# olegroshka/vae-channel-dynamics

Hardware: AMD Instinct MI355X
Metric: images/sec SDXL-VAE train step @256x256 (tracking on) (higher is better)
Workload: dtype f32

## Files before the change

### vae-channel-dynamics_amd/csrc/conv3_upwino.hip

```cpp
#include "wino_common.h"
#include <type_traits>
#include <algorithm>

#ifndef VAE_UPW_PRIO
#define VAE_UPW_PRIO 1
#endif
#ifndef VAE_UPW_XCD_LIMIT
#define VAE_UPW_XCD_LIMIT (4 << 20)
#endif
#ifndef VAE_UPW_X3
#define VAE_UPW_X3 1
#endif
#if VAE_UPW_X3
#include "bf16_frag.h"
#endif

namespace {

constexpr int UTH = 4, UTW = 8;
constexpr int UTL = UTH * UTW;
static_assert(UTL == wino::TILES, "spill_acc");
constexpr int NPOS = 9;
constexpr int UNT = 512;
constexpr int UNB = 2;
constexpr int UHF = (UTH + 2) * (UTW + 2);
constexpr int UHD = (2 * UTH + 2) * (2 * UTW + 2);
constexpr int UMLD = 33;
constexpr int USM = NPOS * UTL * UMLD;

#if !VAE_UPW_X3
constexpr int UBK = 8;
constexpr int USV = NPOS * UTL * UBK;
constexpr int USH = UHD * UBK;
constexpr int UP_LDS = (USM > 2 * USV + 2 * USH ? USM : 2 * USV + 2 * USH) * 4;

__global__ __launch_bounds__(256) void upwino_weights_kernel(const float* __restrict__ W, int N, int K, int dgrad, int64_t sn, int64_t sk, int64_t st,
                                                             float* __restrict__ U) {
  const int64_t i = (int64_t)blockIdx.x * 256 + threadIdx.x;
  if (i >= (int64_t)N * K) return;
  const int k = (int)(i % K), n = (int)(i / K);
  float g[3][3];
  wino::u_gather(W, n, k, dgrad, sn, sk, st, g);
  float t[3][3];
#pragma unroll
  for (int b = 0; b < 3; ++b) {
    t[0][b] = g[0][b];
    t[1][b] = (g[0][b] + g[2][b]) + g[1][b];
    t[2][b] = g[2][b];
  }
  float* o = wino::u_out<NPOS>(U, N, n, k);
#pragma unroll
  for (int a = 0; a < 3; ++a) {
    wino::u_at(o, N, a * 3 + 0) = t[a][0];
    wino::u_at(o, N, a * 3 + 1) = (t[a][0] + t[a][2]) + t[a][1];
    wino::u_at(o, N, a * 3 + 2) = t[a][2];
  }
}

template <bool DG>
__global__ __launch_bounds__(UNT, 4) void conv3_upwino_kernel(vae_igemm_args p, const float* __restrict__ U, int tiles_x, int tiles_y, int xcd_sp) {
  constexpr int WBN = 32 * UNB;
  constexpr int HW_ = DG ? 2 * UTW + 2 : UTW + 2;
  constexpr int HP = DG ? UHD : UHF;
  __shared__ __attribute__((aligned(16))) float wsm[UP_LDS / 4];
  float* const sV = wsm;
  float* const sH = wsm + 2 * USV;

  const int tid = threadIdx.x, lane = tid & 63, wave = tid >> 6;
  const int xw0 = (blockIdx.x & 1) * 2;
  const bool extra = wave == xw0 || wave == xw0 + 1;
  const int xnb = wave - xw0;
  const int lr = lane & 31, lh = lane >> 5;
  const vae_conv_geom g = p.g;
  const int tilesN = (p.N + WBN - 1) / WBN;
  const wino::TileId wg = wino::tile_of_workgroup(blockIdx.x, tilesN, tiles_x, tiles_y, xcd_sp);
  const int b = wg.b;
  const int y0 = wg.ty * UTH, x0 = wg.tx * UTW, n0 = wg.tn * WBN;
  const int nsteps = p.K / UBK;

  const bool hrole = tid < 2 * HP;
  const int hp = tid >> 1, hq = tid & 1;
  const int hy = (DG ? 2 * y0 : y0) - 1 + hp / HW_, hx = (DG ? 2 * x0 : x0) - 1 + hp % HW_;
  const bool hin = hrole && ((unsigned)hy < (unsigned)g.Hs) && ((unsigned)hx < (unsigned)g.Ws);
  const auto rsA = VAE_BUF_RSRC(p.A + (int64_t)b * g.Hs * g.Ws * g.Cs, (size_t)g.Hs * g.Ws * g.Cs * 4u);
  const unsigned hbase = hin ? (unsigned)(((hy * g.Ws + hx) * g.Cs + hq * 4) * 4) : BUF_OOB;
  f32x4 rh = {0.f, 0.f, 0.f, 0.f};
  auto load_halo_into = [&](int step, f32x4& h) {
    const bool ok = hin && step < nsteps;
    h = VAE_BUF_LOAD4(rsA, ok ? hbase + (unsigned)(step * UBK * 4) : BUF_OOB);
  };
  auto store_halo_from = [&](float* dst, const f32x4& h) {
    if (hrole) *reinterpret_cast<f32x4*>(&dst[hp * UBK + hq * 4]) = h;
  };

  const bool vrole = tid < 256;
  const int vt = (tid >> 3) & 31, vc = tid & 7;
  const int vorg = DG ? ((2 * (vt >> 3)) * HW_ + 2 * (vt & 7)) * UBK + vc : ((vt >> 3) * HW_ + (vt & 7)) * UBK + vc;
  auto write_v = [&](const float* sHc, float* dst) {
    if (!vrole) return;
    float r[3][DG ? 4 : 3];
    if (!DG) {
      float d[3][3];
#pragma unroll
      for (int i = 0; i < 3; ++i)
#pragma unroll
        for (int j = 0; j < 3; ++j) d[i][j] = sHc[vorg + (i * HW_ + j) * UBK];
#pragma unroll
      for (int j = 0; j < 3; ++j) {
        r[0][j] = d[0][j] - d[1][j];
        r[1][j] = d[1][j];
        r[2][j] = d[1][j] - d[2][j];
      }
#pragma unroll
      for (int a = 0; a < 3; ++a) {
        dst[((a * 3 + 0) * UTL + vt) * UBK + vc] = r[a][0] - r[a][1];
        dst[((a * 3 + 1) * UTL + vt) * UBK + vc] = r[a][1];
        dst[((a * 3 + 2) * UTL + vt) * UBK + vc] = r[a][1] - r[a][2];
      }
    } else {
      float d[4][4];
#pragma unroll
      for (int i = 0; i < 4; ++i)
#pragma unroll
        for (int j = 0; j < 4; ++j) d[i][j] = sHc[vorg + (i * HW_ + j) * UBK];
#pragma unroll
      for (int j = 0; j < 4; ++j) {
        r[0][j] = d[0][j] - d[2][j];
        r[1][j] = d[1][j] + d[2][j];
        r[2][j] = d[1][j] - d[3][j];
      }
#pragma unroll
      for (int a = 0; a < 3; ++a) {
        dst[((a * 3 + 0) * UTL + vt) * UBK + vc] = r[a][0] - r[a][2];
        dst[((a * 3 + 1) * UTL + vt) * UBK + vc] = r[a][1] + r[a][2];
        dst[((a * 3 + 2) * UTL + vt) * UBK + vc] = r[a][1] - r[a][3];
      }
    }
  };

  const auto rsU = VAE_BUF_RSRC(U, wino::u_bytes(nsteps, NPOS, p.N));
  unsigned bvo[UNB];
#pragma unroll
  for (int q = 0; q < UNB; ++q) bvo[q] = (n0 + q * 32 + lr < p.N) ? wino::u_frag(n0 + q * 32 + lr, lh) : BUF_OOB;
  const unsigned bpos = wino::u_pos_bytes(p.N);
  const unsigned bvx = extra ? bvo[xnb & 1] : BUF_OOB;
  f32x4 bq[UNB + 1];
  auto load_b1 = [&](int step, int i) {
    const int st = min(step, nsteps - 1);
    const unsigned so = __builtin_amdgcn_readfirstlane((unsigned)(st * NPOS + (i < UNB ? wave : 8)) * bpos);
    bq[i] = __builtin_bit_cast(f32x4, __builtin_amdgcn_raw_buffer_load_b128(rsU, i < UNB ? bvo[i < UNB ? i : 0] : bvx, so, 0));
  };

  f32x16 acc[UNB], accx;
#pragma unroll
  for (int nb = 0; nb < UNB; ++nb)
#pragma unroll
    for (int e = 0; e < 16; ++e) acc[nb][e] = 0.f;
#pragma unroll
  for (int e = 0; e < 16; ++e) accx[e] = 0.f;

#pragma unroll
  for (int i = 0; i <= UNB; ++i) load_b1(0, i);
  {
    f32x4 h0, h1;
    load_halo_into(0, h0);
    load_halo_into(1, h1);
    load_halo_into(2, rh);
    store_halo_from(sH, h0);
    store_halo_from(sH + USH, h1);
  }
  __syncthreads();
  write_v(sH, sV);
  __syncthreads();
  auto multiply = [&](const float* cV, int s) {
    const f32x4 a4 = *reinterpret_cast<const f32x4*>(&cV[(wave * UTL + lr) * UBK + 4 * lh]);
    f32x4 ax = a4;
    if (extra) ax = *reinterpret_cast<const f32x4*>(&cV[(8 * UTL + lr) * UBK + 4 * lh]);
#pragma unroll
    for (int nb = 0; nb < UNB; ++nb) {
#pragma unroll
      for (int e = 0; e < 4; ++e) acc[nb] = __builtin_amdgcn_mfma_f32_32x32x2f32(a4[e], bq[nb][e], acc[nb], 0, 0, 0);
      __builtin_amdgcn_sched_barrier(0);
      load_b1(s + 1, nb);
      __builtin_amdgcn_sched_barrier(0);
    }
    if (extra) {
#pragma unroll
      for (int e = 0; e < 4; ++e) accx = __builtin_amdgcn_mfma_f32_32x32x2f32(ax[e], bq[UNB][e], accx, 0, 0, 0);
    }
    __builtin_amdgcn_sched_barrier(0);
    load_b1(s + 1, UNB);
    __builtin_amdgcn_sched_barrier(0);
  };
  auto stage_next = [&](int s, int par) {
    if (s + 1 < nsteps) write_v(sH + (par ^ 1) * USH, sV + (par ^ 1) * USV);
    store_halo_from(sH + par * USH, rh);
    load_halo_into(s + 3, rh);
  };
  auto step = [&](int s, int par, auto first_c) {
    const float* cV = sV + par * USV;
    if (decltype(first_c)::value) {
      stage_next(s, par);
      __builtin_amdgcn_sched_barrier(0);
      multiply(cV, s);
    } else {
      multiply(cV, s);
      __builtin_amdgcn_sched_barrier(0);
      stage_next(s, par);
    }
    __syncthreads();
  };
  auto run = [&](auto first_c) {
    int s = 0;
    for (; s + 1 < nsteps; s += 2) {
      step(s, 0, first_c);
      step(s + 1, 1, first_c);
    }
    if (s < nsteps) step(s, 0, first_c);
  };
#if VAE_UPW_PRIO
  if (DG && __builtin_amdgcn_readfirstlane(tid) >= 256) __builtin_amdgcn_s_setprio(1);
#endif
  if (wave < 4) run(std::true_type{});
  else run(std::false_type{});
#if VAE_UPW_PRIO
  if (DG) __builtin_amdgcn_s_setprio(0);
#endif

  float* const sM = wsm;
  const size_t obytes = (size_t)g.Ho * g.Wo * p.ldc * 4u;
  const auto rsC = VAE_BUF_RSRC(p.C + (int64_t)b * g.Ho * g.Wo * p.ldc, obytes);
#pragma unroll
  for (int nb = 0; nb < UNB; ++nb) {
    if (nb > 0) __syncthreads();
    wino::spill_acc(sM, wave, UMLD, acc[nb], lr, lh);
    if (wave == xw0 + nb) wino::spill_acc(sM, 8, UMLD, accx, lr, lh);
    __syncthreads();
    {
#pragma unroll
      for (int rnd = 0; rnd < 2; ++rnd) {
        const int co = tid & 31, tile = (tid >> 5) + 16 * rnd;
        const int col = n0 + nb * 32 + co;
        float m[9];
#pragma unroll
        for (int pos = 0; pos < 9; ++pos) m[pos] = sM[(pos * UTL + tile) * UMLD + co];
        const int oy = y0 + (tile >> 3), ox = x0 + (tile & 7);
        if (!DG) {
          const float bv = (p.bias && col < p.N) ? p.bias[col] : 0.f;
          float h[2][3];
#pragma unroll
          for (int j = 0; j < 3; ++j) {
            h[0][j] = m[0 * 3 + j] + m[1 * 3 + j];
            h[1][j] = m[1 * 3 + j] - m[2 * 3 + j];
          }
#pragma unroll
          for (int a = 0; a < 2; ++a) {
            const float yv[2] = {h[a][0] + h[a][1], h[a][1] - h[a][2]};
#pragma unroll
            for (int bb = 0; bb < 2; ++bb) {
              const int py = 2 * oy + a, px = 2 * ox + bb;
              const unsigned off = (col < p.N && py < g.Ho && px < g.Wo) ? (unsigned)(((py * g.Wo + px) * p.ldc + col) * 4) : BUF_OOB;
              __builtin_amdgcn_raw_buffer_store_b32(__builtin_bit_cast(unsigned, yv[bb] + bv), rsC, off, 0, 0);
            }
          }
        } else {
          const float h0 = (m[0] + m[3]) - m[6], h1 = (m[1] + m[4]) - m[7], h2 = (m[2] + m[5]) - m[8];
          const float v = (h0 + h1) - h2;
          const unsigned off = (col < p.N && oy < g.Ho && ox < g.Wo) ? (unsigned)(((oy * g.Wo + ox) * p.ldc + col) * 4) : BUF_OOB;
          __builtin_amdgcn_raw_buffer_store_b32(__builtin_bit_cast(unsigned, v), rsC, off, 0, 0);
        }
      }
    }
  }
}

#else
constexpr int XBK = 16;
constexpr int XPL = NPOS * UTL * XBK;
constexpr int XSV = 3 * XPL;
template <bool DG>
constexpr int upw_lds_bytes() {
  constexpr int used = 2 * XSV * 2 + 2 * (DG ? UHD : UHF) * XBK * 4;
  return used > USM * 4 ? used : USM * 4;
}
extern __shared__ __attribute__((aligned(16))) float upw_lds[];

__host__ __device__ __forceinline__ int upw_chunks(int K) { return (K + XBK - 1) / XBK; }
__host__ __device__ __forceinline__ unsigned upw_plane_bytes(int N) { return (unsigned)N * (XBK * 2u); }
__host__ __device__ __forceinline__ size_t upw_u_bytes(int K, int N) { return (size_t)upw_chunks(K) * NPOS * 3 * upw_plane_bytes(N); }

__device__ __forceinline__ void upw_u_transform(const float (&g)[3][3], float (&o)[9]) {
  float t[3][3];
#pragma unroll
  for (int b = 0; b < 3; ++b) {
    t[0][b] = g[0][b];
    t[1][b] = (g[0][b] + g[2][b]) + g[1][b];
    t[2][b] = g[2][b];
  }
#pragma unroll
  for (int a = 0; a < 3; ++a) {
    o[a * 3 + 0] = t[a][0];
    o[a * 3 + 1] = (t[a][0] + t[a][2]) + t[a][1];
    o[a * 3 + 2] = t[a][2];
  }
}

__global__ __launch_bounds__(256) void upwino_weights_kernel(const float* __restrict__ W, int N, int K, int dgrad, int64_t sn, int64_t sk, int64_t st,
                                                             u16* __restrict__ U) {
  const int K16 = upw_chunks(K) * XBK;
  const int64_t i = (int64_t)blockIdx.x * 256 + threadIdx.x;
  if (i >= (int64_t)N * K16) return;
  const int k = (int)(i % K16), n = (int)(i / K16);
  float u[9];
  if (k < K) {
    float g[3][3];
    wino::u_gather(W, n, k, dgrad, sn, sk, st, g);
    upw_u_transform(g, u);
  } else {
#pragma unroll
    for (int pos = 0; pos < 9; ++pos) u[pos] = 0.f;
  }
  u16* o = U + ((int64_t)(k >> 4) * NPOS * 3 * N + n) * XBK + (k & 15);
#pragma unroll
  for (int pos = 0; pos < 9; ++pos) {
    unsigned hi, mid, lo;
    split3_pair(u[pos], 0.f, hi, mid, lo);
    o[(int64_t)(pos * 3 + 0) * N * XBK] = (u16)hi;
    o[(int64_t)(pos * 3 + 1) * N * XBK] = (u16)mid;
    o[(int64_t)(pos * 3 + 2) * N * XBK] = (u16)lo;
  }
}

template <bool DG>
__global__ __launch_bounds__(UNT, 4) void conv3_upwino_kernel(vae_igemm_args p, const u16* __restrict__ U, int tiles_x, int tiles_y, int xcd_sp) {
  constexpr int WBN = 32 * UNB;
  constexpr int HW_ = DG ? 2 * UTW + 2 : UTW + 2;
  constexpr int HP = DG ? UHD : UHF;
  constexpr int XSH = HP * XBK;
  u16* const sV = reinterpret_cast<u16*>(upw_lds);
  float* const sH = upw_lds + XSV;

  const int tid = threadIdx.x, lane = tid & 63, wave = tid >> 6;
  const int xw0 = (blockIdx.x & 1) * 2;
  const bool extra = wave == xw0 || wave == xw0 + 1;
  const int xnb = wave - xw0;
  const int lr = lane & 31, lh = lane >> 5;
  const vae_conv_geom g = p.g;
  const int tilesN = (p.N + WBN - 1) / WBN;
  const wino::TileId wg = wino::tile_of_workgroup(blockIdx.x, tilesN, tiles_x, tiles_y, xcd_sp);
  const int b = wg.b;
  const int y0 = wg.ty * UTH, x0 = wg.tx * UTW, n0 = wg.tn * WBN;
  const int nsteps = upw_chunks(p.K);

  const bool hrole = tid < 2 * HP;
  const int hp = tid >> 1, hq = tid & 1;
  const int hy = (DG ? 2 * y0 : y0) - 1 + hp / HW_, hx = (DG ? 2 * x0 : x0) - 1 + hp % HW_;
  const bool hin = hrole && ((unsigned)hy < (unsigned)g.Hs) && ((unsigned)hx < (unsigned)g.Ws);
  const auto rsA = VAE_BUF_RSRC(p.A + (int64_t)b * g.Hs * g.Ws * g.Cs, (size_t)g.Hs * g.Ws * g.Cs * 4u);
  const unsigned hbase = hin ? (unsigned)(((hy * g.Ws + hx) * g.Cs + hq * 8) * 4) : BUF_OOB;
  f32x4 rh[2] = {{0.f, 0.f, 0.f, 0.f}, {0.f, 0.f, 0.f, 0.f}};
  auto load_halo_into = [&](int step, f32x4 (&h)[2]) {
    const bool ok = hin && step * XBK + hq * 8 < p.K;
    h[0] = VAE_BUF_LOAD4(rsA, ok ? hbase + (unsigned)(step * XBK * 4) : BUF_OOB);
    h[1] = VAE_BUF_LOAD4(rsA, ok ? hbase + (unsigned)(step * XBK * 4 + 16) : BUF_OOB);
  };
  auto store_halo_from = [&](float* dst, const f32x4 (&h)[2]) {
    if (hrole) {
      *reinterpret_cast<f32x4*>(&dst[hp * XBK + hq * 8]) = h[0];
      *reinterpret_cast<f32x4*>(&dst[hp * XBK + hq * 8 + 4]) = h[1];
    }
  };

  const bool vrole = tid < 256;
  const int vt = (tid >> 3) & 31, vc = tid & 7;
  const int vorg = DG ? ((2 * (vt >> 3)) * HW_ + 2 * (vt & 7)) * XBK + 2 * vc : ((vt >> 3) * HW_ + (vt & 7)) * XBK + 2 * vc;
  const int vdst = vt * XBK + (((vc >> 2) ^ ((vt >> 3) & 1)) * 8) + (vc & 3) * 2;
  auto write_v = [&](const float* sHc, u16* dst) __attribute__((always_inline)) {
    if (!vrole) return;
    typedef float f32x2 __attribute__((ext_vector_type(2)));
    constexpr int NJ = DG ? 4 : 3;
#pragma unroll
    for (int a = 0; a < 3; ++a) {
      const int ia = DG ? (a == 0 ? 0 : 1) : (a == 0 ? 0 : 1), ib = DG ? (a == 2 ? 3 : 2) : (a == 0 ? 1 : 2);
      float r[NJ][2];
#pragma unroll
      for (int j = 0; j < NJ; ++j) {
        const f32x2 x = *reinterpret_cast<const f32x2*>(&sHc[vorg + (ia * HW_ + j) * XBK]);
        if (!DG && a == 1) {
          r[j][0] = x[0];
          r[j][1] = x[1];
        } else {
          const f32x2 y = *reinterpret_cast<const f32x2*>(&sHc[vorg + (ib * HW_ + j) * XBK]);
          const bool add = DG && a == 1;
          r[j][0] = add ? x[0] + y[0] : x[0] - y[0];
          r[j][1] = add ? x[1] + y[1] : x[1] - y[1];
        }
      }
      float o[3][2];
#pragma unroll
      for (int c = 0; c < 2; ++c) {
        if (!DG) {
          o[0][c] = r[0][c] - r[1][c];
          o[1][c] = r[1][c];
          o[2][c] = r[1][c] - r[2][c];
        } else {
          o[0][c] = r[0][c] - r[2][c];
          o[1][c] = r[1][c] + r[2][c];
          o[2][c] = r[1][c] - r[NJ - 1][c];
        }
      }
#pragma unroll
      for (int bb = 0; bb < 3; ++bb) {
        const int pos = a * 3 + bb;
        unsigned hi, mid, lo;
        split3_pair(o[bb][0], o[bb][1], hi, mid, lo);
        *reinterpret_cast<unsigned*>(&dst[0 * XPL + pos * UTL * XBK + vdst]) = hi;
        *reinterpret_cast<unsigned*>(&dst[1 * XPL + pos * UTL * XBK + vdst]) = mid;
        *reinterpret_cast<unsigned*>(&dst[2 * XPL + pos * UTL * XBK + vdst]) = lo;
      }
    }
  };

  const auto rsU = VAE_BUF_RSRC(U, upw_u_bytes(p.K, p.N));
  unsigned bvo[UNB];
#pragma unroll
  for (int q = 0; q < UNB; ++q) bvo[q] = (n0 + q * 32 + lr < p.N) ? (unsigned)(((n0 + q * 32 + lr) * XBK + lh * 8) * 2) : BUF_OOB;
  const unsigned bpl = upw_plane_bytes(p.N);
  const unsigned bvx = extra ? bvo[xnb & 1] : BUF_OOB;
  bf16x8 bq[UNB + 1][3];
  auto load_b3 = [&](int step, int i) __attribute__((always_inline)) {
    const int st = min(step, nsteps - 1);
    const unsigned so = __builtin_amdgcn_readfirstlane((unsigned)((st * NPOS + (i < UNB ? wave : 8)) * 3) * bpl);
#pragma unroll
    for (int pl = 0; pl < 3; ++pl)
      bq[i][pl] = __builtin_bit_cast(bf16x8, __builtin_amdgcn_raw_buffer_load_b128(rsU, i < UNB ? bvo[i < UNB ? i : 0] : bvx, so + (unsigned)pl * bpl, 0));
  };

  f32x16 acc[UNB], accx;
#pragma unroll
  for (int nb = 0; nb < UNB; ++nb)
#pragma unroll
    for (int e = 0; e < 16; ++e) acc[nb][e] = 0.f;
#pragma unroll
  for (int e = 0; e < 16; ++e) accx[e] = 0.f;

#pragma unroll
  for (int i = 0; i <= UNB; ++i) load_b3(0, i);
  {
    f32x4 h0[2], h1[2];
    load_halo_into(0, h0);
    load_halo_into(1, h1);
    load_halo_into(2, rh);
    store_halo_from(sH, h0);
    store_halo_from(sH + XSH, h1);
  }
  __syncthreads();
  write_v(sH, sV);
  __syncthreads();
  const int afrag = lr * XBK + ((lh ^ ((lr >> 3) & 1)) * 8);
  auto multiply = [&](const u16* cV, int s) __attribute__((always_inline)) {
    bf16x8 a[3];
#pragma unroll
    for (int pl = 0; pl < 3; ++pl) a[pl] = frag_direct(&cV[pl * XPL + wave * UTL * XBK + afrag]);
#pragma unroll
    for (int nb = 0; nb < UNB; ++nb) {
#pragma unroll
      for (int t = 0; t < 6; ++t) acc[nb] = mma_x3_term(t, a, bq[nb], acc[nb]);
      __builtin_amdgcn_sched_barrier(0);
      load_b3(s + 1, nb);
      __builtin_amdgcn_sched_barrier(0);
    }
    if (extra) {
#pragma unroll
      for (int pl = 0; pl < 3; ++pl) a[pl] = frag_direct(&cV[pl * XPL + 8 * UTL * XBK + afrag]);
#pragma unroll
      for (int t = 0; t < 6; ++t) accx = mma_x3_term(t, a, bq[UNB], accx);
    }
    __builtin_amdgcn_sched_barrier(0);
    load_b3(s + 1, UNB);
    __builtin_amdgcn_sched_barrier(0);
  };
  auto stage_next = [&](int s, int par) __attribute__((always_inline)) {
    store_halo_from(sH + par * XSH, rh);
    if (s + 1 < nsteps) write_v(sH + (par ^ 1) * XSH, sV + (par ^ 1) * XSV);
    load_halo_into(s + 3, rh);
  };
  auto step = [&](int s, int par, auto first_c) __attribute__((always_inline)) {
    const u16* cV = sV + par * XSV;
    if (decltype(first_c)::value) {
      stage_next(s, par);
      __builtin_amdgcn_sched_barrier(0);
      multiply(cV, s);
    } else {
      multiply(cV, s);
      __builtin_amdgcn_sched_barrier(0);
      stage_next(s, par);
    }
    __syncthreads();
  };
  auto run = [&](auto first_c) __attribute__((always_inline)) {
    int s = 0;
    for (; s + 1 < nsteps; s += 2) {
      step(s, 0, first_c);
      step(s + 1, 1, first_c);
    }
    if (s < nsteps) step(s, 0, first_c);
  };
#if VAE_UPW_PRIO
  if (DG && __builtin_amdgcn_readfirstlane(tid) >= 256) __builtin_amdgcn_s_setprio(1);
#endif
  if (wave < 4) run(std::true_type{});
  else run(std::false_type{});
#if VAE_UPW_PRIO
  if (DG) __builtin_amdgcn_s_setprio(0);
#endif

  float* const sM = upw_lds;
  const size_t obytes = (size_t)g.Ho * g.Wo * p.ldc * 4u;
  const auto rsC = VAE_BUF_RSRC(p.C + (int64_t)b * g.Ho * g.Wo * p.ldc, obytes);
#pragma unroll
  for (int nb = 0; nb < UNB; ++nb) {
    if (nb > 0) __syncthreads();
    wino::spill_acc(sM, wave, UMLD, acc[nb], lr, lh);
    if (wave == xw0 + nb) wino::spill_acc(sM, 8, UMLD, accx, lr, lh);
    __syncthreads();
    {
#pragma unroll
      for (int rnd = 0; rnd < 2; ++rnd) {
        const int co = tid & 31, tile = (tid >> 5) + 16 * rnd;
        const int col = n0 + nb * 32 + co;
        float m[9];
#pragma unroll
        for (int pos = 0; pos < 9; ++pos) m[pos] = sM[(pos * UTL + tile) * UMLD + co];
        const int oy = y0 + (tile >> 3), ox = x0 + (tile & 7);
        if (!DG) {
          const float bv = (p.bias && col < p.N) ? p.bias[col] : 0.f;
          float h[2][3];
#pragma unroll
          for (int j = 0; j < 3; ++j) {
            h[0][j] = m[0 * 3 + j] + m[1 * 3 + j];
            h[1][j] = m[1 * 3 + j] - m[2 * 3 + j];
          }
#pragma unroll
          for (int a = 0; a < 2; ++a) {
            const float yv[2] = {h[a][0] + h[a][1], h[a][1] - h[a][2]};
#pragma unroll
            for (int bb = 0; bb < 2; ++bb) {
              const int py = 2 * oy + a, px = 2 * ox + bb;
              const unsigned off = (col < p.N && py < g.Ho && px < g.Wo) ? (unsigned)(((py * g.Wo + px) * p.ldc + col) * 4) : BUF_OOB;
              __builtin_amdgcn_raw_buffer_store_b32(__builtin_bit_cast(unsigned, yv[bb] + bv), rsC, off, 0, 0);
            }
          }
        } else {
          const float h0 = (m[0] + m[3]) - m[6], h1 = (m[1] + m[4]) - m[7], h2 = (m[2] + m[5]) - m[8];
          const float v = (h0 + h1) - h2;
          const unsigned off = (col < p.N && oy < g.Ho && ox < g.Wo) ? (unsigned)(((oy * g.Wo + ox) * p.ldc + col) * 4) : BUF_OOB;
          __builtin_amdgcn_raw_buffer_store_b32(__builtin_bit_cast(unsigned, v), rsC, off, 0, 0);
        }
      }
    }
  }
}
#endif

}

bool conv3_upwino_eligible(const vae_igemm_args& a) {
  const vae_conv_geom& g = a.g;
  if (!wino::conv_eligible_common(a, NPOS) || a.xf != VAE_XF_NONE) return false;
  if (a.track != nullptr || a.res != nullptr || a.gstat != nullptr || a.a_bf16 || a.res_bf16) return false;
  int Hl, Wl;
  if (g.mode == VAE_MODE_UP2X) {
    if (g.Ho != 2 * g.Hs || g.Wo != 2 * g.Ws || a.sk != 1) return false;
    Hl = g.Hs; Wl = g.Ws;
  } else if (g.mode == VAE_MODE_UP2X_DGRAD) {
    if (g.Hs != 2 * g.Ho || g.Ws != 2 * g.Wo || a.sn != 1 || a.bias != nullptr) return false;
    Hl = g.Ho; Wl = g.Wo;
  } else {
    return false;
  }
  if (Hl % UTH != 0 || Wl % UTW != 0 || a.K % 8 != 0 || a.K < 64 || a.K > 1024 || a.N < 32 || a.N % 4 != 0 || g.Cs < a.K) return false;
#if VAE_UPW_X3
  if (upw_u_bytes(a.K, a.N) >= BUF_MAX) return false;
#endif
  return true;
}

int64_t conv3_upwino_weight_bytes(const vae_igemm_args& a) {
#if VAE_UPW_X3
  return (int64_t)upw_u_bytes(a.K, a.N);
#else
  return (int64_t)wino::u_bytes(a.K / UBK, NPOS, a.N);
#endif
}

int launch_upwino_weights(const vae_igemm_args& a, float* U, hipStream_t st) {
#if VAE_UPW_X3
  const int64_t n = (int64_t)a.N * upw_chunks(a.K) * XBK;
  hipLaunchKernelGGL(upwino_weights_kernel, dim3((unsigned)((n + 255) / 256)), dim3(256), 0, st, a.W, a.N, a.K, a.g.mode == VAE_MODE_UP2X_DGRAD ? 1 : 0,
                     a.sn, a.sk, a.st, reinterpret_cast<u16*>(U));
  return 0;
#else
  return wino::launch_weights(upwino_weights_kernel, a, a.g.mode == VAE_MODE_UP2X_DGRAD, U, st);
#endif
}

int launch_conv3_upwino(const vae_igemm_args& a, const float* U, hipStream_t st) {
  const vae_conv_geom& g = a.g;
  const bool dg = g.mode == VAE_MODE_UP2X_DGRAD;
  const int Hl = dg ? g.Ho : g.Hs, Wl = dg ? g.Wo : g.Ws;
  const int tx = Wl / UTW, ty = Hl / UTH;
  const int tilesN = (a.N + 32 * UNB - 1) / (32 * UNB);
  const int64_t nt = (int64_t)tilesN * tx * ty * g.B;
  if (nt > 0x7fffffffLL) return VAE_EINVAL;
  constexpr size_t xcd_u = (size_t)VAE_UPW_XCD_LIMIT;
  const int xcd_sp = wino::xcd_spatial(tilesN, (size_t)conv3_upwino_weight_bytes(a), xcd_u, (int64_t)tx * ty * g.B);
#if VAE_UPW_X3
  const u16* Up = reinterpret_cast<const u16*>(U);
  if (dg) {
    VAE_RESERVE_LDS(conv3_upwino_kernel<true>, upw_lds_bytes<true>(), "conv3_upwino");
    hipLaunchKernelGGL((conv3_upwino_kernel<true>), dim3((unsigned)nt), dim3(UNT), upw_lds_bytes<true>(), st, a, Up, tx, ty, xcd_sp);
  } else {
    VAE_RESERVE_LDS(conv3_upwino_kernel<false>, upw_lds_bytes<false>(), "conv3_upwino");
    hipLaunchKernelGGL((conv3_upwino_kernel<false>), dim3((unsigned)nt), dim3(UNT), upw_lds_bytes<false>(), st, a, Up, tx, ty, xcd_sp);
  }
#else
  if (dg) hipLaunchKernelGGL((conv3_upwino_kernel<true>), dim3((unsigned)nt), dim3(UNT), 0, st, a, U, tx, ty, xcd_sp);
  else hipLaunchKernelGGL((conv3_upwino_kernel<false>), dim3((unsigned)nt), dim3(UNT), 0, st, a, U, tx, ty, xcd_sp);
#endif
  return 0;
}
```

Measured before the change: 118.8.

## Widen upsample Winograd conv N-tile to four 32-column blocks per workgroup

Makes the number of 32-wide output-channel blocks per workgroup configurable and defaults both forward and dgrad to 4 instead of 2. Each workgroup now reuses its transformed input tile across twice as many output channels, which halves the number of workgroups along N and cuts redundant input halo loads and V transforms. Waves 4-7 take the ninth Winograd position for the extra blocks, and partially live N tiles are masked. In exchange, accumulator register pressure doubles, so launch bounds drop to 2 blocks per CU, and fewer workgroups may reduce occupancy and parallelism on small layers.

New measurement: 120.5, median of 6. +1.5%, better.

```diff
diff --git a/vae-channel-dynamics_amd/csrc/conv3_upwino.hip b/vae-channel-dynamics_amd/csrc/conv3_upwino.hip
--- a/vae-channel-dynamics_amd/csrc/conv3_upwino.hip
+++ b/vae-channel-dynamics_amd/csrc/conv3_upwino.hip
@@ -10,6 +10,12 @@
 #endif
 #ifndef VAE_UPW_X3
 #define VAE_UPW_X3 1
+#endif
+#ifndef VAE_UPW_NB_FWD
+#define VAE_UPW_NB_FWD 4
+#endif
+#ifndef VAE_UPW_NB_DG
+#define VAE_UPW_NB_DG 4
 #endif
 #if VAE_UPW_X3
 #include "bf16_frag.h"
@@ -279,6 +285,11 @@
 constexpr int XPL = NPOS * UTL * XBK;
 constexpr int XSV = 3 * XPL;
 template <bool DG>
+constexpr int upw_nb() {
+  return DG ? VAE_UPW_NB_DG : VAE_UPW_NB_FWD;
+}
+static_assert((upw_nb<false>() == 2 || upw_nb<false>() == 4) && (upw_nb<true>() == 2 || upw_nb<true>() == 4), "VAE_UPW_NB_*: 2 or 4");
+template <bool DG>
 constexpr int upw_lds_bytes() {
   constexpr int used = 2 * XSV * 2 + 2 * (DG ? UHD : UHF) * XBK * 4;
   return used > USM * 4 ? used : USM * 4;
@@ -332,8 +343,10 @@
 }
 
 template <bool DG>
-__global__ __launch_bounds__(UNT, 4) void conv3_upwino_kernel(vae_igemm_args p, const u16* __restrict__ U, int tiles_x, int tiles_y, int xcd_sp) {
-  constexpr int WBN = 32 * UNB;
+__global__ __launch_bounds__(UNT, upw_nb<DG>() > 2 ? 2 : 4) void conv3_upwino_kernel(vae_igemm_args p, const u16* __restrict__ U, int tiles_x, int tiles_y, int xcd_sp) {
+  constexpr int NB = upw_nb<DG>();
+  constexpr bool WIDE = NB > 2;
+  constexpr int WBN = 32 * NB;
   constexpr int HW_ = DG ? 2 * UTW + 2 : UTW + 2;
   constexpr int HP = DG ? UHD : UHF;
   constexpr int XSH = HP * XBK;
@@ -341,9 +354,6 @@
   float* const sH = upw_lds + XSV;
 
   const int tid = threadIdx.x, lane = tid & 63, wave = tid >> 6;
-  const int xw0 = (blockIdx.x & 1) * 2;
-  const bool extra = wave == xw0 || wave == xw0 + 1;
-  const int xnb = wave - xw0;
   const int lr = lane & 31, lh = lane >> 5;
   const vae_conv_geom g = p.g;
   const int tilesN = (p.N + WBN - 1) / WBN;
@@ -351,6 +361,10 @@
   const int b = wg.b;
   const int y0 = wg.ty * UTH, x0 = wg.tx * UTW, n0 = wg.tn * WBN;
   const int nsteps = upw_chunks(p.K);
+  const int nlive = WIDE ? min(NB, (p.N - n0 + 31) >> 5) : NB;
+  const int xw0 = WIDE ? 4 : (blockIdx.x & 1) * 2;
+  const int xnb = wave - xw0;
+  const bool extra = WIDE ? (wave >= 4 && xnb < nlive) : (wave == xw0 || wave == xw0 + 1);
 
   const bool hrole = tid < 2 * HP;
   const int hp = tid >> 1, hq = tid & 1;
@@ -422,30 +436,31 @@
   };
 
   const auto rsU = VAE_BUF_RSRC(U, upw_u_bytes(p.K, p.N));
-  unsigned bvo[UNB];
-#pragma unroll
-  for (int q = 0; q < UNB; ++q) bvo[q] = (n0 + q * 32 + lr < p.N) ? (unsigned)(((n0 + q * 32 + lr) * XBK + lh * 8) * 2) : BUF_OOB;
+  unsigned bvo[NB];
+#pragma unroll
+  for (int q = 0; q < NB; ++q) bvo[q] = (n0 + q * 32 + lr < p.N) ? (unsigned)(((n0 + q * 32 + lr) * XBK + lh * 8) * 2) : BUF_OOB;
   const unsigned bpl = upw_plane_bytes(p.N);
-  const unsigned bvx = extra ? bvo[xnb & 1] : BUF_OOB;
-  bf16x8 bq[UNB + 1][3];
+  const unsigned bvw = (n0 + xnb * 32 + lr < p.N) ? (unsigned)(((n0 + xnb * 32 + lr) * XBK + lh * 8) * 2) : BUF_OOB;
+  const unsigned bvx = extra ? (WIDE ? bvw : bvo[xnb & 1]) : BUF_OOB;
+  bf16x8 bq[NB + 1][3];
   auto load_b3 = [&](int step, int i) __attribute__((always_inline)) {
     const int st = min(step, nsteps - 1);
-    const unsigned so = __builtin_amdgcn_readfirstlane((unsigned)((st * NPOS + (i < UNB ? wave : 8)) * 3) * bpl);
+    const unsigned so = __builtin_amdgcn_readfirstlane((unsigned)((st * NPOS + (i < NB ? wave : 8)) * 3) * bpl);
 #pragma unroll
     for (int pl = 0; pl < 3; ++pl)
-      bq[i][pl] = __builtin_bit_cast(bf16x8, __builtin_amdgcn_raw_buffer_load_b128(rsU, i < UNB ? bvo[i < UNB ? i : 0] : bvx, so + (unsigned)pl * bpl, 0));
-  };
-
-  f32x16 acc[UNB], accx;
-#pragma unroll
-  for (int nb = 0; nb < UNB; ++nb)
+      bq[i][pl] = __builtin_bit_cast(bf16x8, __builtin_amdgcn_raw_buffer_load_b128(rsU, i < NB ? bvo[i < NB ? i : 0] : bvx, so + (unsigned)pl * bpl, 0));
+  };
+
+  f32x16 acc[NB], accx;
+#pragma unroll
+  for (int nb = 0; nb < NB; ++nb)
 #pragma unroll
     for (int e = 0; e < 16; ++e) acc[nb][e] = 0.f;
 #pragma unroll
   for (int e = 0; e < 16; ++e) accx[e] = 0.f;
 
 #pragma unroll
-  for (int i = 0; i <= UNB; ++i) load_b3(0, i);
+  for (int i = 0; i <= NB; ++i) load_b3(0, i);
   {
     f32x4 h0[2], h1[2];
     load_halo_into(0, h0);
@@ -463,9 +478,11 @@
 #pragma unroll
     for (int pl = 0; pl < 3; ++pl) a[pl] = frag_direct(&cV[pl * XPL + wave * UTL * XBK + afrag]);
 #pragma unroll
-    for (int nb = 0; nb < UNB; ++nb) {
-#pragma unroll
-      for (int t = 0; t < 6; ++t) acc[nb] = mma_x3_term(t, a, bq[nb], acc[nb]);
+    for (int nb = 0; nb < NB; ++nb) {
+      if (!WIDE || nb < nlive) {
+#pragma unroll
+        for (int t = 0; t < 6; ++t) acc[nb] = mma_x3_term(t, a, bq[nb], acc[nb]);
+      }
       __builtin_amdgcn_sched_barrier(0);
       load_b3(s + 1, nb);
       __builtin_amdgcn_sched_barrier(0);
@@ -474,10 +491,10 @@
 #pragma unroll
       for (int pl = 0; pl < 3; ++pl) a[pl] = frag_direct(&cV[pl * XPL + 8 * UTL * XBK + afrag]);
 #pragma unroll
-      for (int t = 0; t < 6; ++t) accx = mma_x3_term(t, a, bq[UNB], accx);
+      for (int t = 0; t < 6; ++t) accx = mma_x3_term(t, a, bq[NB], accx);
     }
     __builtin_amdgcn_sched_barrier(0);
-    load_b3(s + 1, UNB);
+    load_b3(s + 1, NB);
     __builtin_amdgcn_sched_barrier(0);
   };
   auto stage_next = [&](int s, int par) __attribute__((always_inline)) {
@@ -519,7 +536,8 @@
   const size_t obytes = (size_t)g.Ho * g.Wo * p.ldc * 4u;
   const auto rsC = VAE_BUF_RSRC(p.C + (int64_t)b * g.Ho * g.Wo * p.ldc, obytes);
 #pragma unroll
-  for (int nb = 0; nb < UNB; ++nb) {
+  for (int nb = 0; nb < NB; ++nb) {
+    if (WIDE && nb >= nlive) break;
     if (nb > 0) __syncthreads();
     wino::spill_acc(sM, wave, UMLD, acc[nb], lr, lh);
     if (wave == xw0 + nb) wino::spill_acc(sM, 8, UMLD, accx, lr, lh);
@@ -610,7 +628,12 @@
   const bool dg = g.mode == VAE_MODE_UP2X_DGRAD;
   const int Hl = dg ? g.Ho : g.Hs, Wl = dg ? g.Wo : g.Ws;
   const int tx = Wl / UTW, ty = Hl / UTH;
-  const int tilesN = (a.N + 32 * UNB - 1) / (32 * UNB);
+#if VAE_UPW_X3
+  const int wbn = 32 * (dg ? upw_nb<true>() : upw_nb<false>());
+#else
+  const int wbn = 32 * UNB;
+#endif
+  const int tilesN = (a.N + wbn - 1) / wbn;
   const int64_t nt = (int64_t)tilesN * tx * ty * g.B;
   if (nt > 0x7fffffffLL) return VAE_EINVAL;
   constexpr size_t xcd_u = (size_t)VAE_UPW_XCD_LIMIT;
```
